# dhansmair/flamingo-mini

Hardware: AMD Instinct MI355X
Metric: images/sec (fwd+bwd) flamingo-mini bs=32 (higher is better)
Workload: dtype bf16

## Files before the change

### flamingo-mini_amd/csrc/ff_rowwise.hip

```cpp
#include "ff_common.h"
#include "ff_internal.h"

namespace ff {

#ifdef FF_XA_TIMELINE
__device__ unsigned long long g_ln_timeline[4096 * 8];
#define FF_LTL(i) do { if (threadIdx.x == 0 && blockIdx.x < 4096) g_ln_timeline[blockIdx.x * 8 + (i)] = __builtin_amdgcn_s_memrealtime(); } while (0)
#else
#define FF_LTL(i) do { } while (0)
#endif

template <typename T, int VEC> FF_DEV void ld(const T* p, float (&o)[VEC]) {
    if constexpr (VEC == 1) o[0] = to_f32(p[0]);
    else Vec<T>::load(p, o);
}
template <typename T, int VEC> FF_DEV void st(T* p, const float (&o)[VEC]) {
    if constexpr (VEC == 1) p[0] = from_f32<T>(o[0]);
    else Vec<T>::store(p, o);
}

template <typename T, int VEC>
__global__ __launch_bounds__(256) void ln_fwd_kernel(const LnArgs a_in, const T* __restrict__ x, const T* __restrict__ add,
                                                     const T* __restrict__ gamma, const T* __restrict__ beta, T* __restrict__ y,
                                                     float* __restrict__ mean, float* __restrict__ rstd) {
    const LnArgs a = fetch_args(a_in);
    pin_args(x, add, gamma, beta, y, mean, rstd);
    const int lane = threadIdx.x & 63;
    const int row = blockIdx.x * 4 + (threadIdx.x >> 6);
    if (row >= a.rows) return;
    const T* xr = x + a.x_map.off(row);
    const T* ar = nullptr;
    if (add) ar = add + (long long)((row % a.add_rows_per_seg) / a.add_div) * a.cols;
    const int nchunk = a.cols / VEC;
    float mu, rs;
    if (nchunk <= 4 * 64 && VEC > 1) {
        float v[4][VEC];
#pragma unroll
        for (int u = 0; u < 4; u++) {
            const int c = lane + 64 * u;
            if (c < nchunk) {
                ld<T, VEC>(xr + c * VEC, v[u]);
                if (ar) {
                    float t[VEC];
                    ld<T, VEC>(ar + c * VEC, t);
#pragma unroll
                    for (int i = 0; i < VEC; i++) v[u][i] += t[i];
                }
            }
        }
        if (a.stats_given) {
            mu = mean[row];
            rs = rstd[row];
        } else {
            float s = 0.f;
#pragma unroll
            for (int u = 0; u < 4; u++)
                if (lane + 64 * u < nchunk)
#pragma unroll
                    for (int i = 0; i < VEC; i++) s += v[u][i];
            mu = wave_sum(s) / (float)a.cols;
            float q = 0.f;
#pragma unroll
            for (int u = 0; u < 4; u++)
                if (lane + 64 * u < nchunk)
#pragma unroll
                    for (int i = 0; i < VEC; i++) q += (v[u][i] - mu) * (v[u][i] - mu);
            rs = rsqrtf(wave_sum(q) / (float)a.cols + a.eps);
            if (lane == 0 && mean) {
                mean[row] = mu;
                rstd[row] = rs;
            }
        }
        if (!y) return;
        T* yr = y + a.y_map.off(row);
#pragma unroll
        for (int u = 0; u < 4; u++) {
            const int c = lane + 64 * u;
            if (c < nchunk) {
                float g[VEC], b[VEC], o[VEC];
                ld<T, VEC>(gamma + c * VEC, g);
                ld<T, VEC>(beta + c * VEC, b);
#pragma unroll
                for (int i = 0; i < VEC; i++) o[i] = (v[u][i] - mu) * rs * g[i] + b[i];
                st<T, VEC>(yr + c * VEC, o);
            }
        }
        return;
    }
    if (a.stats_given) {
        mu = mean[row];
        rs = rstd[row];
    } else {
        float s = 0.f;
        for (int c = lane; c < nchunk; c += 64) {
            float v[VEC];
            ld<T, VEC>(xr + c * VEC, v);
            if (ar) {
                float t[VEC];
                ld<T, VEC>(ar + c * VEC, t);
#pragma unroll
                for (int i = 0; i < VEC; i++) v[i] += t[i];
            }
#pragma unroll
            for (int i = 0; i < VEC; i++) s += v[i];
        }
        mu = wave_sum(s) / (float)a.cols;
        float q = 0.f;
        for (int c = lane; c < nchunk; c += 64) {
            float v[VEC];
            ld<T, VEC>(xr + c * VEC, v);
            if (ar) {
                float t[VEC];
                ld<T, VEC>(ar + c * VEC, t);
#pragma unroll
                for (int i = 0; i < VEC; i++) v[i] += t[i];
            }
#pragma unroll
            for (int i = 0; i < VEC; i++) q += (v[i] - mu) * (v[i] - mu);
        }
        rs = rsqrtf(wave_sum(q) / (float)a.cols + a.eps);
        if (lane == 0 && mean) {
            mean[row] = mu;
            rstd[row] = rs;
        }
    }
    if (!y) return;
    T* yr = y + a.y_map.off(row);
    for (int c = lane; c < nchunk; c += 64) {
        float v[VEC], g[VEC], b[VEC];
        ld<T, VEC>(xr + c * VEC, v);
        if (ar) {
            float t[VEC];
            ld<T, VEC>(ar + c * VEC, t);
#pragma unroll
            for (int i = 0; i < VEC; i++) v[i] += t[i];
        }
        ld<T, VEC>(gamma + c * VEC, g);
        ld<T, VEC>(beta + c * VEC, b);
#pragma unroll
        for (int i = 0; i < VEC; i++) v[i] = (v[i] - mu) * rs * g[i] + b[i];
        st<T, VEC>(yr + c * VEC, v);
    }
}

template <typename T, int VEC>
__global__ __launch_bounds__(256) void ln_bwd_dx_kernel(const LnArgs a_in, const T* __restrict__ dy, const T* __restrict__ x,
                                                        const T* __restrict__ add, const T* __restrict__ gamma,
                                                        const float* __restrict__ mean, const float* __restrict__ rstd, T* dx,
                                                        const T* dx_res) {
    const LnArgs a = fetch_args(a_in);
    pin_args(dy, x, add, gamma, mean, rstd, dx, dx_res);
    const int lane = threadIdx.x & 63;
    const int row = blockIdx.x * 4 + (threadIdx.x >> 6);
    if (row >= a.rows) return;
    const T* xr = x + a.x_map.off(row);
    const T* dyr = dy + a.y_map.off(row);
    const T* ar = nullptr;
    if (add) ar = add + (long long)((row % a.add_rows_per_seg) / a.add_div) * a.cols;
    const float mu = mean[row], rs = rstd[row];
    const int nchunk = a.cols / VEC;
    float s1 = 0.f, s2 = 0.f;
    for (int c = lane; c < nchunk; c += 64) {
        float v[VEC], d[VEC], g[VEC];
        ld<T, VEC>(xr + c * VEC, v);
        if (ar) {
            float t[VEC];
            ld<T, VEC>(ar + c * VEC, t);
#pragma unroll
            for (int i = 0; i < VEC; i++) v[i] += t[i];
        }
        ld<T, VEC>(dyr + c * VEC, d);
        ld<T, VEC>(gamma + c * VEC, g);
#pragma unroll
        for (int i = 0; i < VEC; i++) {
            const float dyh = d[i] * g[i];
            s1 += dyh;
            s2 += dyh * (v[i] - mu) * rs;
        }
    }
    const float m1 = wave_sum(s1) / (float)a.cols, m2 = wave_sum(s2) / (float)a.cols;
    const long long doff = a.dx_map.off(row);
    for (int c = lane; c < nchunk; c += 64) {
        float v[VEC], d[VEC], g[VEC], o[VEC];
        ld<T, VEC>(xr + c * VEC, v);
        if (ar) {
            float t[VEC];
            ld<T, VEC>(ar + c * VEC, t);
#pragma unroll
            for (int i = 0; i < VEC; i++) v[i] += t[i];
        }
        ld<T, VEC>(dyr + c * VEC, d);
        ld<T, VEC>(gamma + c * VEC, g);
#pragma unroll
        for (int i = 0; i < VEC; i++) o[i] = rs * (d[i] * g[i] - m1 - (v[i] - mu) * rs * m2);
        if (dx_res) {
            float q[VEC];
            ld<T, VEC>(dx_res + doff + c * VEC, q);
#pragma unroll
            for (int i = 0; i < VEC; i++) o[i] += q[i];
        }
        st<T, VEC>(dx + doff + c * VEC, o);
    }
}


template <typename T, int VEC, int NCH>
__global__ __launch_bounds__(256) void ln_bwd_fused_kernel(const LnArgs a_in, const T* __restrict__ dy, const T* __restrict__ x,
                                                           const T* __restrict__ add, const T* __restrict__ gamma,
                                                           const float* __restrict__ mean, const float* __restrict__ rstd, T* dx,
                                                           const T* dx_res, const T* __restrict__ dot_a, const T* __restrict__ dot_b,
                                                           float* __restrict__ partial, int rows_per_block) {
    FF_LTL(0);
    const LnArgs a = fetch_args(a_in);
    pin_args(dy, x, add, gamma, mean, rstd, dx, dx_res, dot_a, dot_b, partial, rows_per_block);
    extern __shared__ __attribute__((aligned(16))) float sacc[];
    FF_LTL(1);
    __shared__ float red[4];
    const int lane = threadIdx.x & 63, w = threadIdx.x >> 6;
    const int nchunk = a.cols / VEC;
    float accg[NCH][VEC], accb[NCH][VEC];
#pragma unroll
    for (int i = 0; i < NCH; i++)
#pragma unroll
        for (int e = 0; e < VEC; e++) accg[i][e] = accb[i][e] = 0.f;
    float da = 0.f, db = 0.f;
    const int row_end = min(a.rows, (int)(blockIdx.x + 1) * rows_per_block);
    auto load_dy = [&](int row, const T* dyr, int c, float (&d)[VEC]) {
        if (a.dy_splits > 0) {
            const float* pp = (const float*)dy + (long long)row * a.cols + c * VEC;
#pragma unroll
            for (int e = 0; e < VEC; e++) d[e] = 0.f;
            for (int sp = 0; sp < a.dy_splits; sp++) {
#pragma unroll
                for (int e = 0; e < VEC; e += 4) {
                    const f32x4 q = *(const f32x4*)(pp + (long long)sp * a.dy_slab + e);
                    d[e] += q[0]; d[e + 1] += q[1]; d[e + 2] += q[2]; d[e + 3] += q[3];
                }
            }
        } else ld<T, VEC>(dyr + c * VEC, d);
    };
    for (int row = blockIdx.x * rows_per_block + w; row < row_end; row += 4) {
        const T* xr = x + a.x_map.off(row);
        const T* dyr = a.dy_splits > 0 ? dy : dy + a.y_map.off(row);
        const T* ar = add ? add + (long long)((row % a.add_rows_per_seg) / a.add_div) * a.cols : nullptr;
        const float mu = mean[row], rs = rstd[row];
        float s1 = 0.f, s2 = 0.f;
        constexpr bool KEEP = NCH <= 4;
        constexpr bool HOIST = KEEP && VEC > 1;
        float xk[KEEP ? NCH : 1][VEC], dk[KEEP ? NCH : 1][VEC];
        uint4 rq[HOIST ? NCH : 1], ra[HOIST ? NCH : 1], rb[HOIST ? NCH : 1];
        const long long doff = a.dx_map.off(row);
#pragma unroll
        for (int i = 0; i < NCH; i++) {
            const int c = lane + 64 * i;
            if (c < nchunk) {
                float v[VEC], d[VEC], g[VEC];
                ld<T, VEC>(xr + c * VEC, v);
                if (ar) {
                    float t[VEC];
                    ld<T, VEC>(ar + c * VEC, t);
#pragma unroll
                    for (int e = 0; e < VEC; e++) v[e] += t[e];
                }
                load_dy(row, dyr, c, d);
                ld<T, VEC>(gamma + c * VEC, g);
                if constexpr (HOIST) {
                    if (dx_res) rq[i] = *(const uint4*)(dx_res + doff + c * VEC);
                    if (dot_a) ra[i] = *(const uint4*)(dot_a + doff + c * VEC);
                    if (dot_b) rb[i] = *(const uint4*)(dot_b + doff + c * VEC);
                }
#pragma unroll
                for (int e = 0; e < VEC; e++) {
                    const float dyh = d[e] * g[e], xh = (v[e] - mu) * rs;
                    s1 += dyh;
                    s2 += dyh * xh;
                    if (KEEP) { xk[i][e] = xh; dk[i][e] = d[e]; }
                }
            }
        }
        const float m1 = wave_sum(s1) / (float)a.cols, m2 = wave_sum(s2) / (float)a.cols;
        auto unpack = [](const uint4& r, float (&o)[VEC]) {
            if constexpr (VEC > 1) {
                typedef typename Vec<T>::raw raw_t;
                const raw_t x = __builtin_bit_cast(raw_t, r);
#pragma unroll
                for (int e = 0; e < VEC; e++) o[e] = to_f32(x[e]);
            }
        };
#pragma unroll
        for (int i = 0; i < NCH; i++) {
            const int c = lane + 64 * i;
            if (c < nchunk) {
                float xh[VEC], d[VEC], g[VEC], o[VEC];
                if (KEEP) {
#pragma unroll
                    for (int e = 0; e < VEC; e++) { xh[e] = xk[i][e]; d[e] = dk[i][e]; }
                } else {
                    float v[VEC];
                    ld<T, VEC>(xr + c * VEC, v);
                    if (ar) {
                        float t[VEC];
                        ld<T, VEC>(ar + c * VEC, t);
#pragma unroll
                        for (int e = 0; e < VEC; e++) v[e] += t[e];
                    }
                    load_dy(row, dyr, c, d);
#pragma unroll
                    for (int e = 0; e < VEC; e++) xh[e] = (v[e] - mu) * rs;
                }
                ld<T, VEC>(gamma + c * VEC, g);
#pragma unroll
                for (int e = 0; e < VEC; e++) {
                    o[e] = rs * (d[e] * g[e] - m1 - xh[e] * m2);
                    accg[i][e] += d[e] * xh[e];
                    accb[i][e] += d[e];
                }
                if (dx_res) {
                    float q[VEC];
                    if constexpr (HOIST) unpack(rq[i], q);
                    else ld<T, VEC>(dx_res + doff + c * VEC, q);
                    if (dot_a) {
                        float u[VEC];
                        if constexpr (HOIST) unpack(ra[i], u);
                        else ld<T, VEC>(dot_a + doff + c * VEC, u);
#pragma unroll
                        for (int e = 0; e < VEC; e++) da += q[e] * u[e];
                    }
#pragma unroll
                    for (int e = 0; e < VEC; e++) o[e] += q[e];
                }
                if (dx) {
                    float r[VEC];
#pragma unroll
                    for (int e = 0; e < VEC; e++) r[e] = to_f32(from_f32<T>(o[e]));
                    if (dot_b) {
                        float u[VEC];
                        if constexpr (HOIST) unpack(rb[i], u);
                        else ld<T, VEC>(dot_b + doff + c * VEC, u);
#pragma unroll
                        for (int e = 0; e < VEC; e++) db += r[e] * u[e];
                    }
                    st<T, VEC>(dx + doff + c * VEC, o);
                }
            }
        }
    }
    FF_LTL(2);
    {
        float* mine = sacc + (size_t)w * 2 * a.cols;
#pragma unroll
        for (int i = 0; i < NCH; i++) {
            const int c = lane + 64 * i;
            if (c < nchunk) {
#pragma unroll
                for (int e = 0; e < VEC; e += 4) {
                    *(f32x4*)(mine + c * VEC + e) = f32x4{accg[i][e], accg[i][e + 1], accg[i][e + 2], accg[i][e + 3]};
                    *(f32x4*)(mine + a.cols + c * VEC + e) = f32x4{accb[i][e], accb[i][e + 1], accb[i][e + 2], accb[i][e + 3]};
                }
            }
        }
    }
    __syncthreads();
    FF_LTL(3);
    const long long P = 2LL * a.cols + 2;
    float* out = partial + (long long)blockIdx.x * P;
    for (int i = threadIdx.x * 4; i < 2 * a.cols; i += 256 * 4) {
        const f32x4 s0 = *(const f32x4*)(sacc + i), s1 = *(const f32x4*)(sacc + 2 * a.cols + i);
        const f32x4 s2 = *(const f32x4*)(sacc + 4 * a.cols + i), s3 = *(const f32x4*)(sacc + 6 * a.cols + i);
        float* o = out + i;
        o[0] = (s0[0] + s1[0]) + (s2[0] + s3[0]); o[1] = (s0[1] + s1[1]) + (s2[1] + s3[1]);
        o[2] = (s0[2] + s1[2]) + (s2[2] + s3[2]); o[3] = (s0[3] + s1[3]) + (s2[3] + s3[3]);
    }
    da = block_sum<4>(da, red);
    db = block_sum<4>(db, red);
    if (threadIdx.x == 0) { out[2 * a.cols] = da; out[2 * a.cols + 1] = db; }
    FF_LTL(4);
}

template <typename T>
FF_DEV void ln_final_body(int nblk, int cols, const float* __restrict__ partial, T* dgamma, T* dbeta, const T* alpha_a, T* out_a, const T* alpha_b,
                          T* out_b) {
    __shared__ float red[16][17];
    const int P = 2 * cols + 2;
    const int tx = threadIdx.x & 15, ty = threadIdx.x >> 4;
    const int idx = blockIdx.x * 16 + tx;
    float v[8] = {0.f, 0.f, 0.f, 0.f, 0.f, 0.f, 0.f, 0.f};
    if (idx < P) {
        int b = ty;
        for (; b + 7 * 16 < nblk; b += 8 * 16) {
#pragma unroll
            for (int u = 0; u < 8; u++) v[u] += partial[(long long)(b + 16 * u) * P + idx];
        }
        for (; b < nblk; b += 16) v[0] += partial[(long long)b * P + idx];
    }
    red[ty][tx] = ((v[0] + v[1]) + (v[2] + v[3])) + ((v[4] + v[5]) + (v[6] + v[7]));
    __syncthreads();
    if (ty == 0 && idx < P) {
        float s = 0.f;
#pragma unroll
        for (int u = 0; u < 16; u++) s += red[u][tx];
        const float v = s;
        if (idx < cols) { if (dgamma) dgamma[idx] = from_f32<T>(v); }
        else if (idx < 2 * cols) { if (dbeta) dbeta[idx - cols] = from_f32<T>(v); }
        else if (idx == 2 * cols) {
            if (out_a) { const float t = tanhf(to_f32(alpha_a[0])); out_a[0] = from_f32<T>(v * (1.f - t * t)); }
        } else if (out_b) { const float t = tanhf(to_f32(alpha_b[0])); out_b[0] = from_f32<T>(v * (1.f - t * t)); }
    }
}
template <typename T>
__global__ __launch_bounds__(256) void ln_bwd_final_kernel(int nblk, int cols, const float* __restrict__ partial, T* dgamma, T* dbeta,
                                                           const T* alpha_a, T* out_a, const T* alpha_b, T* out_b) {
    pin_args(nblk, cols, partial, dgamma, dbeta, alpha_a, out_a, alpha_b, out_b);
    ln_final_body<T>(nblk, cols, partial, dgamma, dbeta, alpha_a, out_a, alpha_b, out_b);
}
struct LnFinishTable {
    LnPending s[kLnFinishMax];
};
template <typename T>
__global__ __launch_bounds__(256) void ln_bwd_final_multi_kernel(const LnFinishTable t) {
    const LnPending& e = t.s[blockIdx.y];
    if ((int)blockIdx.x * 16 >= 2 * e.cols + 2) return;
    ln_final_body<T>(e.nblk, e.cols, e.partial, (T*)e.dgamma, (T*)e.dbeta, (const T*)e.alpha_a, (T*)e.out_a, (const T*)e.alpha_b, (T*)e.out_b);
}

struct ColReduceArgs {
    int rows, cols;
// ... 131 lines not shown

int gate_grad(int dtype, int rows, int cols, const void* a, const void* b, const void* alpha, void* dalpha, void* ws,
              size_t ws_bytes, hipStream_t st_);

static bool vec_ok(int dtype, int cols, std::initializer_list<RowMap> maps, std::initializer_list<const void*> ptrs) {
    const int n = dtype == FF_DTYPE_BF16 ? 8 : 4;
    if (cols % n) return false;
    for (const RowMap& m : maps)
        if (m.ld % n || (m.rows_per_seg > 0 && m.seg_stride % n)) return false;
    for (const void* p : ptrs)
        if (p && (uintptr_t)p % 16) return false;
    return true;
}

#define FF_DISPATCH_T_VEC(dtype, vec, ...)                 \
    do {                                                    \
        if ((dtype) == FF_DTYPE_BF16) {                     \
            typedef bf16 T;                                 \
            if (vec) { constexpr int VEC = 8; __VA_ARGS__; }       \
            else { constexpr int VEC = 1; __VA_ARGS__; }           \
        } else {                                            \
            typedef float T;                                \
            if (vec) { constexpr int VEC = 4; __VA_ARGS__; }       \
            else { constexpr int VEC = 1; __VA_ARGS__; }           \
        }                                                   \
    } while (0)

int layernorm_fwd(const LnArgs& a, const void* x, const void* add, const void* gamma, const void* beta, void* y, float* mean,
                  float* rstd, hipStream_t st_) {
    FF_CHECK(a.rows > 0 && a.cols > 0 && x, FF_ERR_SHAPE, "layernorm_fwd: bad shape rows=%d cols=%d", a.rows, a.cols);
    FF_CHECK(!a.stats_given || (mean && rstd), FF_ERR_SHAPE, "layernorm_fwd: stats_given without statistics");
    FF_CHECK(!y || (gamma && beta), FF_ERR_SHAPE, "layernorm_fwd: gamma/beta missing");
    FF_CHECK(!add || (a.add_rows_per_seg > 0 && a.add_div > 0), FF_ERR_SHAPE, "layernorm_fwd: addend needs add_rows_per_seg/add_div");
    const bool v = vec_ok(a.dtype, a.cols, {a.x_map, a.y_map}, {x, add, gamma, beta, y});
    const int grid = cdiv(a.rows, 4);
    FF_DISPATCH_T_VEC(a.dtype, v, ln_fwd_kernel<T, VEC><<<dim3(grid), dim3(256), 0, st_>>>(a, (const T*)x, (const T*)add, (const T*)gamma, (const T*)beta, (T*)y, mean, rstd));
    return check_launch("ln_fwd");
}

static void split_plan(int n_rows_in_group, int col_blocks, int ngroups, int& rows_per_split, int& nsplit) {
    int target = std::max(1, 512 / std::max(1, col_blocks * ngroups));
    nsplit = std::max(1, std::min(std::min(target, 32), cdiv(n_rows_in_group, 32)));
    rows_per_split = cdiv(n_rows_in_group, nsplit);
    nsplit = cdiv(n_rows_in_group, rows_per_split);
}

static size_t col_reduce_ws(int n_rows_in_group, int cols, int ngroups, int nslots) {
    int rps, ns;
    split_plan(n_rows_in_group, 1, ngroups, rps, ns);
    return (size_t)ns * ngroups * nslots * cols * sizeof(float);
}


static int ln_fused_blocks(int rows, int& rows_per_block) {
    rows_per_block = std::max(4, (cdiv(rows, 256) + 3) / 4 * 4);
    return cdiv(rows, rows_per_block);
}
static bool ln_fused_ok(int dtype, int cols, bool vec) {
    if (!vec) return false;
    const int n = dtype == FF_DTYPE_BF16 ? 8 : 4;
    return cdiv(cols / n, 64) <= 8 && (size_t)8 * cols * sizeof(float) <= 150 * 1024;
}
size_t layernorm_bwd_workspace(int rows, int cols) {
    int rpb;
    const size_t fused = (size_t)ln_fused_blocks(rows, rpb) * (2 * (size_t)cols + 2) * sizeof(float);
    return std::max(fused, col_reduce_ws(rows, cols, 1, 2));
}

bool layernorm_bwd_deferrable(int dtype, int cols) { return cols % (dtype == FF_DTYPE_BF16 ? 8 : 4) == 0 && ln_fused_ok(dtype, cols, true); }
int layernorm_bwd_partial_blocks(int rows) {
    int rpb;
    return ln_fused_blocks(rows, rpb);
}
size_t layernorm_bwd_partial_bytes(int rows, int cols) { return (size_t)layernorm_bwd_partial_blocks(rows) * (2 * (size_t)cols + 2) * sizeof(float); }

template <typename T, int VEC>
static int launch_ln_fused(const LnArgs& a, const void* dy, const void* x, const void* add, const void* gamma, const float* mean,
                           const float* rstd, void* dx, const void* dx_res, const LnDots& dots, void* dgamma, void* dbeta, float* partial,
                           hipStream_t st_, LnPending* pending) {
    int rpb;
    const int nblk = ln_fused_blocks(a.rows, rpb);
    const int nch = cdiv(a.cols / VEC, 64);
    const size_t lds = (size_t)8 * a.cols * sizeof(float);
#define FF_LN_LAUNCH(NCH)                                                                                                                 \
    do {                                                                                                                                  \
        if (lds > 48 * 1024) {                                                                                                            \
            static bool attr[64] = {};                                                                                                    \
            int dev = 0;                                                                                                                  \
            (void)hipGetDevice(&dev);                                                                                                     \
            if (dev < 0 || dev >= 64 || !attr[dev]) {                                                                                     \
                hipFuncSetAttribute((const void*)ln_bwd_fused_kernel<T, VEC, NCH>, hipFuncAttributeMaxDynamicSharedMemorySize, 150 * 1024); \
                if (dev >= 0 && dev < 64) attr[dev] = true;                                                                               \
            }                                                                                                                             \
        }                                                                                                                                 \
        ln_bwd_fused_kernel<T, VEC, NCH><<<dim3(nblk), dim3(256), lds, st_>>>(a, (const T*)dy, (const T*)x, (const T*)add, (const T*)gamma, \
                                                                              mean, rstd, (T*)dx, (const T*)dx_res, (const T*)dots.a,     \
                                                                              (const T*)dots.b, partial, rpb);                            \
    } while (0)
    if (nch <= 2) FF_LN_LAUNCH(2);
    else if (nch <= 4) FF_LN_LAUNCH(4);
    else FF_LN_LAUNCH(8);
#undef FF_LN_LAUNCH
    FF_TRY(check_launch("ln_bwd_fused"));
    if (pending) {
        pending->partial = partial; pending->nblk = nblk; pending->cols = a.cols; pending->dgamma = dgamma; pending->dbeta = dbeta;
        pending->alpha_a = dots.alpha_a; pending->out_a = dots.out_a; pending->alpha_b = dots.alpha_b; pending->out_b = dots.out_b;
        return FF_OK;
    }
    const int P = 2 * a.cols + 2;
    ln_bwd_final_kernel<T><<<dim3(cdiv(P, 16)), dim3(256), 0, st_>>>(nblk, a.cols, partial, (T*)dgamma, (T*)dbeta, (const T*)dots.alpha_a,
                                                                     (T*)dots.out_a, (const T*)dots.alpha_b, (T*)dots.out_b);
    return check_launch("ln_bwd_final");
}

int layernorm_bwd(const LnArgs& a, const void* dy, const void* x, const void* add, const void* gamma, const float* mean,
                  const float* rstd, void* dx, const void* dx_residual, void* dgamma, void* dbeta, void* ws, size_t ws_bytes,
                  hipStream_t st_, const LnDots* dots_in, LnPending* pending) {
    FF_CHECK(a.rows > 0 && a.cols > 0 && dy && x && gamma && mean && rstd, FF_ERR_SHAPE, "layernorm_bwd: null/shape");
    if (pending) *pending = LnPending{};
    FF_CHECK(!add || (a.add_rows_per_seg > 0 && a.add_div > 0), FF_ERR_SHAPE, "layernorm_bwd: addend needs add_rows_per_seg/add_div");
    const LnDots dots = dots_in ? *dots_in : LnDots{};
    FF_CHECK(!dots.a || dx_residual, FF_ERR_SHAPE, "layernorm_bwd: dot_a is taken against dx_residual");
    FF_CHECK(!dots.b || dx, FF_ERR_SHAPE, "layernorm_bwd: dot_b is taken against dx");
    const bool v = vec_ok(a.dtype, a.cols, {a.x_map, a.y_map, a.dx_map}, {x, add, gamma, dy, dx, dx_residual, dots.a, dots.b});
    FF_CHECK(a.dy_splits == 0 || (ln_fused_ok(a.dtype, a.cols, v) && (dgamma || dots.a || dots.b) && a.cols % 4 == 0), FF_ERR_UNSUPPORTED,
             "layernorm_bwd: summing split-K slabs needs the one-pass kernel");
    if (ln_fused_ok(a.dtype, a.cols, v) && (dgamma || dots.a || dots.b)) {
        FF_CHECK(!dgamma == !dbeta, FF_ERR_SHAPE, "layernorm_bwd: dgamma and dbeta come together");
        int rpb;
        const size_t need = (size_t)ln_fused_blocks(a.rows, rpb) * (2 * (size_t)a.cols + 2) * sizeof(float);
        FF_CHECK(ws && ws_bytes >= need, FF_ERR_WORKSPACE, "layernorm_bwd workspace: need %zu have %zu", need, ws_bytes);
        if (a.dtype == FF_DTYPE_BF16) return launch_ln_fused<bf16, 8>(a, dy, x, add, gamma, mean, rstd, dx, dx_residual, dots, dgamma, dbeta, (float*)ws, st_, pending);
        return launch_ln_fused<float, 4>(a, dy, x, add, gamma, mean, rstd, dx, dx_residual, dots, dgamma, dbeta, (float*)ws, st_, pending);
    }
    if (dots.a) FF_TRY(gate_grad(a.dtype, a.rows, a.cols, dx_residual, dots.a, dots.alpha_a, dots.out_a, ws, ws_bytes, st_));
    if (dx) {
        const int grid = cdiv(a.rows, 4);
        FF_DISPATCH_T_VEC(a.dtype, v, ln_bwd_dx_kernel<T, VEC><<<dim3(grid), dim3(256), 0, st_>>>(a, (const T*)dy, (const T*)x, (const T*)add, (const T*)gamma, mean, rstd, (T*)dx, (const T*)dx_residual));
        FF_TRY(check_launch("ln_bwd_dx"));
    }
    if (dgamma || dbeta) {
        FF_CHECK(dgamma && dbeta, FF_ERR_SHAPE, "layernorm_bwd: dgamma and dbeta come together");
        const int vecn = v ? (a.dtype == FF_DTYPE_BF16 ? 8 : 4) : 1;
        ColReduceArgs c = {};
        c.rows = a.rows; c.cols = a.cols; c.x_map = a.x_map; c.y_map = a.y_map;
        c.rows_per_batch = a.rows; c.rows_per_group = a.rows; c.n_batch = 1; c.ngroups = 1;
        c.add_rows_per_seg = a.add_rows_per_seg; c.add_div = a.add_div;
        const int col_blocks = cdiv(a.cols, 64 * vecn);
        split_plan(a.rows, col_blocks, 1, c.rows_per_split, c.nsplit);
        const size_t need = (size_t)c.nsplit * 2 * a.cols * sizeof(float);
        FF_CHECK(ws && ws_bytes >= need, FF_ERR_WORKSPACE, "layernorm_bwd workspace: need %zu have %zu", need, ws_bytes);
        FF_DISPATCH_T_VEC(a.dtype, v, col_reduce_kernel<T, VEC, 1><<<dim3(col_blocks, 1, c.nsplit), dim3(256), 0, st_>>>(c, (const T*)x, (const T*)dy, (const T*)add, mean, rstd, (float*)ws));
        FF_TRY(check_launch("ln_bwd_param_partial"));
        const int grid = std::min(cdiv(2LL * a.cols, 256), 1024);
        if (a.dtype == FF_DTYPE_BF16)
            hipLaunchKernelGGL(col_reduce_final_kernel<bf16>, dim3(grid), dim3(256), 0, st_, c.nsplit, 1, 2, a.cols, (const float*)ws, (bf16*)dgamma, (bf16*)dbeta);
        else
            hipLaunchKernelGGL(col_reduce_final_kernel<float>, dim3(grid), dim3(256), 0, st_, c.nsplit, 1, 2, a.cols, (const float*)ws, (float*)dgamma, (float*)dbeta);
        FF_TRY(check_launch("ln_bwd_param_final"));
    }
    if (dots.b) FF_TRY(gate_grad(a.dtype, a.rows, a.cols, dx, dots.b, dots.alpha_b, dots.out_b, ws, ws_bytes, st_));
    return FF_OK;
}

int layernorm_bwd_finish(int dtype, const LnPending* sets, int n, hipStream_t st_) {
    for (int i0 = 0; i0 < n; i0 += kLnFinishMax) {
        LnFinishTable t = {};
        int cnt = 0, pmax = 0;
        for (int i = i0; i < n && i < i0 + kLnFinishMax; i++)
            if (sets[i].partial) {
                t.s[cnt++] = sets[i];
                pmax = std::max(pmax, 2 * sets[i].cols + 2);
            }
        if (!cnt) continue;
        const dim3 grid(cdiv(pmax, 16), cnt);
        if (dtype == FF_DTYPE_BF16) ln_bwd_final_multi_kernel<bf16><<<grid, dim3(256), 0, st_>>>(t);
        else ln_bwd_final_multi_kernel<float><<<grid, dim3(256), 0, st_>>>(t);
        FF_TRY(check_launch("ln_bwd_final_multi"));
    }
    return FF_OK;
}

size_t rows_reduce_workspace(int rows, int cols, int rows_per_batch, int rows_per_group) {
    if (rows_per_batch <= 0 || rows_per_group <= 0) return 0;
// ... 115 lines not shown
```

Measured before the change: 782.3.

## Use buffer loads with OOB masking and batched prefetch in layernorm kernels

```diff
diff --git a/flamingo-mini_amd/csrc/ff_rowwise.hip b/flamingo-mini_amd/csrc/ff_rowwise.hip
--- a/flamingo-mini_amd/csrc/ff_rowwise.hip
+++ b/flamingo-mini_amd/csrc/ff_rowwise.hip
@@ -19,12 +19,160 @@
     else Vec<T>::store(p, o);
 }
 
+typedef __attribute__((ext_vector_type(4))) unsigned u32x4;
+constexpr unsigned kRowOob = 0x80000000u;
+FF_DEV __amdgpu_buffer_rsrc_t row_rsrc(const void* p, bool there = true) { return __builtin_amdgcn_make_buffer_rsrc((void*)p, 0, there ? 0x7fffffff : 0, 0x00020000); }
+FF_DEV u32x4 row_ld(__amdgpu_buffer_rsrc_t r, unsigned byte_off) { return __builtin_amdgcn_raw_buffer_load_b128(r, byte_off, 0, 0); }
+FF_DEV float row_ld_f32(__amdgpu_buffer_rsrc_t r, unsigned byte_off) { return __builtin_bit_cast(float, __builtin_amdgcn_raw_buffer_load_b32(r, byte_off, 0, 0)); }
+FF_DEV int wave_id() { return __builtin_amdgcn_readfirstlane(threadIdx.x >> 6); }
+template <typename T, int VEC> FF_DEV void unpk(const u32x4& r, float (&o)[VEC]) {
+    typedef typename Vec<T>::raw raw_t;
+    const raw_t x = __builtin_bit_cast(raw_t, r);
+#pragma unroll
+    for (int e = 0; e < VEC; e++) o[e] = to_f32(x[e]);
+}
+template <typename T, int VEC> FF_DEV void row_st(__amdgpu_buffer_rsrc_t r, unsigned byte_off, const float (&o)[VEC]) {
+    typename Vec<T>::raw v;
+#pragma unroll
+    for (int e = 0; e < VEC; e++) v[e] = from_f32<T>(o[e]);
+    __builtin_amdgcn_raw_buffer_store_b128(__builtin_bit_cast(u32x4, v), r, byte_off, 0, 0);
+}
+template <typename T, int VEC> FF_DEV void ldb(__amdgpu_buffer_rsrc_t r, int c, float (&o)[VEC]) { unpk<T, VEC>(row_ld(r, (unsigned)c * 16u), o); }
+
+template <typename T, int VEC>
+FF_DEV void ln_fwd_vec(const LnArgs& a, const T* x, const T* add, const T* gamma, const T* beta, T* y, float* mean, float* rstd) {
+    const int lane = threadIdx.x & 63;
+    const int row = blockIdx.x * 4 + wave_id();
+    if (row >= a.rows) return;
+    const bool has_add = add != nullptr;
+    const __amdgpu_buffer_rsrc_t rx = row_rsrc(x + a.x_map.off(row));
+    const __amdgpu_buffer_rsrc_t ra = row_rsrc(add + (long long)((row % (has_add ? a.add_rows_per_seg : 1)) / (has_add ? a.add_div : 1)) * a.cols, has_add);
+    const __amdgpu_buffer_rsrc_t rg = row_rsrc(gamma, y != nullptr), rb = row_rsrc(beta, y != nullptr);
+    const int nchunk = a.cols / VEC;
+    float mu, rs;
+    if (nchunk <= 4 * 64) {
+        u32x4 px[4], pa[4], pg[4], pb[4];
+        bool in[4];
+        unsigned coff[4];
+#pragma unroll
+        for (int u = 0; u < 4; u++) {
+            in[u] = lane + 64 * u < nchunk;
+            coff[u] = in[u] ? (unsigned)(lane + 64 * u) * 16u : kRowOob;
+            px[u] = row_ld(rx, coff[u]);
+        }
+#pragma unroll
+        for (int u = 0; u < 4; u++) pa[u] = row_ld(ra, coff[u]);
+        const float mu_in = row_ld_f32(row_rsrc(mean, a.stats_given != 0), (unsigned)row * 4u);
+        const float rs_in = row_ld_f32(row_rsrc(rstd, a.stats_given != 0), (unsigned)row * 4u);
+#pragma unroll
+        for (int u = 0; u < 4; u++) {
+            pg[u] = row_ld(rg, coff[u]);
+            pb[u] = row_ld(rb, coff[u]);
+        }
+        __builtin_amdgcn_sched_barrier(0);
+        asm volatile("" ::"v"(mu_in), "v"(rs_in));
+        float v[4][VEC];
+#pragma unroll
+        for (int u = 0; u < 4; u++) {
+            float t[VEC];
+            unpk<T, VEC>(px[u], v[u]);
+            unpk<T, VEC>(pa[u], t);
+#pragma unroll
+            for (int i = 0; i < VEC; i++) v[u][i] = has_add ? v[u][i] + t[i] : v[u][i];
+        }
+        if (a.stats_given) {
+            mu = mu_in;
+            rs = rs_in;
+        } else {
+            float s = 0.f;
+#pragma unroll
+            for (int u = 0; u < 4; u++)
+#pragma unroll
+                for (int i = 0; i < VEC; i++) s += v[u][i];
+            mu = wave_sum(s) / (float)a.cols;
+            float q = 0.f;
+#pragma unroll
+            for (int u = 0; u < 4; u++) {
+                const float mu_u = in[u] ? mu : 0.f;
+#pragma unroll
+                for (int i = 0; i < VEC; i++) q += (v[u][i] - mu_u) * (v[u][i] - mu_u);
+            }
+            rs = rsqrtf(wave_sum(q) / (float)a.cols + a.eps);
+            if (lane == 0 && mean) {
+                mean[row] = mu;
+                rstd[row] = rs;
+            }
+        }
+        if (!y) return;
+        const __amdgpu_buffer_rsrc_t ry = row_rsrc(y + a.y_map.off(row));
+#pragma unroll
+        for (int u = 0; u < 4; u++) {
+            float g[VEC], b[VEC], o[VEC];
+            unpk<T, VEC>(pg[u], g);
+            unpk<T, VEC>(pb[u], b);
+#pragma unroll
+            for (int i = 0; i < VEC; i++) o[i] = (v[u][i] - mu) * rs * g[i] + b[i];
+            if (in[u]) row_st<T, VEC>(ry, coff[u], o);
+        }
+        return;
+    }
+    auto load_x = [&](int c, float (&v)[VEC]) {
+        ldb<T, VEC>(rx, c, v);
+        if (has_add) {
+            float t[VEC];
+            ldb<T, VEC>(ra, c, t);
+#pragma unroll
+            for (int i = 0; i < VEC; i++) v[i] += t[i];
+        }
+    };
+    if (a.stats_given) {
+        mu = row_ld_f32(row_rsrc(mean), (unsigned)row * 4u);
+        rs = row_ld_f32(row_rsrc(rstd), (unsigned)row * 4u);
+    } else {
+        float s = 0.f;
+        for (int c = lane; c < nchunk; c += 64) {
+            float v[VEC];
+            load_x(c, v);
+#pragma unroll
+            for (int i = 0; i < VEC; i++) s += v[i];
+        }
+        mu = wave_sum(s) / (float)a.cols;
+        float q = 0.f;
+        for (int c = lane; c < nchunk; c += 64) {
+            float v[VEC];
+            load_x(c, v);
+#pragma unroll
+            for (int i = 0; i < VEC; i++) q += (v[i] - mu) * (v[i] - mu);
+        }
+        rs = rsqrtf(wave_sum(q) / (float)a.cols + a.eps);
+        if (lane == 0 && mean) {
+            mean[row] = mu;
+            rstd[row] = rs;
+        }
+    }
+    if (!y) return;
+    const __amdgpu_buffer_rsrc_t ry = row_rsrc(y + a.y_map.off(row));
+    for (int c = lane; c < nchunk; c += 64) {
+        float v[VEC], g[VEC], b[VEC];
+        load_x(c, v);
+        ldb<T, VEC>(rg, c, g);
+        ldb<T, VEC>(rb, c, b);
+#pragma unroll
+        for (int i = 0; i < VEC; i++) v[i] = (v[i] - mu) * rs * g[i] + b[i];
+        row_st<T, VEC>(ry, (unsigned)c * 16u, v);
+    }
+}
+
 template <typename T, int VEC>
 __global__ __launch_bounds__(256) void ln_fwd_kernel(const LnArgs a_in, const T* __restrict__ x, const T* __restrict__ add,
                                                      const T* __restrict__ gamma, const T* __restrict__ beta, T* __restrict__ y,
                                                      float* __restrict__ mean, float* __restrict__ rstd) {
     const LnArgs a = fetch_args(a_in);
     pin_args(x, add, gamma, beta, y, mean, rstd);
+    if constexpr (VEC > 1) {
+        ln_fwd_vec<T, VEC>(a, x, add, gamma, beta, y, mean, rstd);
+        return;
+    }
     const int lane = threadIdx.x & 63;
     const int row = blockIdx.x * 4 + (threadIdx.x >> 6);
     if (row >= a.rows) return;
@@ -33,60 +181,6 @@
     if (add) ar = add + (long long)((row % a.add_rows_per_seg) / a.add_div) * a.cols;
     const int nchunk = a.cols / VEC;
     float mu, rs;
-    if (nchunk <= 4 * 64 && VEC > 1) {
-        float v[4][VEC];
-#pragma unroll
-        for (int u = 0; u < 4; u++) {
-            const int c = lane + 64 * u;
-            if (c < nchunk) {
-                ld<T, VEC>(xr + c * VEC, v[u]);
-                if (ar) {
-                    float t[VEC];
-                    ld<T, VEC>(ar + c * VEC, t);
-#pragma unroll
-                    for (int i = 0; i < VEC; i++) v[u][i] += t[i];
-                }
-            }
-        }
-        if (a.stats_given) {
-            mu = mean[row];
-            rs = rstd[row];
-        } else {
-            float s = 0.f;
-#pragma unroll
-            for (int u = 0; u < 4; u++)
-                if (lane + 64 * u < nchunk)
-#pragma unroll
-                    for (int i = 0; i < VEC; i++) s += v[u][i];
-            mu = wave_sum(s) / (float)a.cols;
-            float q = 0.f;
-#pragma unroll
-            for (int u = 0; u < 4; u++)
-                if (lane + 64 * u < nchunk)
-#pragma unroll
-                    for (int i = 0; i < VEC; i++) q += (v[u][i] - mu) * (v[u][i] - mu);
-            rs = rsqrtf(wave_sum(q) / (float)a.cols + a.eps);
-            if (lane == 0 && mean) {
-                mean[row] = mu;
-                rstd[row] = rs;
-            }
-        }
-        if (!y) return;
-        T* yr = y + a.y_map.off(row);
-#pragma unroll
-        for (int u = 0; u < 4; u++) {
-            const int c = lane + 64 * u;
-            if (c < nchunk) {
-                float g[VEC], b[VEC], o[VEC];
-                ld<T, VEC>(gamma + c * VEC, g);
-                ld<T, VEC>(beta + c * VEC, b);
-#pragma unroll
-                for (int i = 0; i < VEC; i++) o[i] = (v[u][i] - mu) * rs * g[i] + b[i];
-                st<T, VEC>(yr + c * VEC, o);
-            }
-        }
-        return;
-    }
     if (a.stats_given) {
         mu = mean[row];
         rs = rstd[row];
@@ -150,6 +244,50 @@
                                                         const T* dx_res) {
     const LnArgs a = fetch_args(a_in);
     pin_args(dy, x, add, gamma, mean, rstd, dx, dx_res);
+    if constexpr (VEC > 1) {
+        const int lane = threadIdx.x & 63;
+        const int row = blockIdx.x * 4 + wave_id();
+        if (row >= a.rows) return;
+        const bool has_add = add != nullptr, has_res = dx_res != nullptr;
+        const __amdgpu_buffer_rsrc_t rx = row_rsrc(x + a.x_map.off(row)), rdy = row_rsrc(dy + a.y_map.off(row)), rg = row_rsrc(gamma);
+        const __amdgpu_buffer_rsrc_t ra = row_rsrc(add + (long long)((row % (has_add ? a.add_rows_per_seg : 1)) / (has_add ? a.add_div : 1)) * a.cols, has_add);
+        const long long doff = a.dx_map.off(row);
+        const __amdgpu_buffer_rsrc_t rq = row_rsrc(dx_res + doff, has_res), ro = row_rsrc(dx + doff);
+        const float mu = row_ld_f32(row_rsrc(mean), (unsigned)row * 4u), rs = row_ld_f32(row_rsrc(rstd), (unsigned)row * 4u);
+        const int nchunk = a.cols / VEC;
+        float s1 = 0.f, s2 = 0.f;
+        for (int c = lane; c < nchunk; c += 64) {
+            float v[VEC], t[VEC], d[VEC], g[VEC];
+            ldb<T, VEC>(rx, c, v);
+            ldb<T, VEC>(ra, c, t);
+            ldb<T, VEC>(rdy, c, d);
+            ldb<T, VEC>(rg, c, g);
+#pragma unroll
+            for (int i = 0; i < VEC; i++) {
+                v[i] = has_add ? v[i] + t[i] : v[i];
+                const float dyh = d[i] * g[i];
+                s1 += dyh;
+                s2 += dyh * (v[i] - mu) * rs;
+            }
+        }
+        const float m1 = wave_sum(s1) / (float)a.cols, m2 = wave_sum(s2) / (float)a.cols;
+        for (int c = lane; c < nchunk; c += 64) {
+            float v[VEC], t[VEC], d[VEC], g[VEC], q[VEC], o[VEC];
+            ldb<T, VEC>(rx, c, v);
+            ldb<T, VEC>(ra, c, t);
+            ldb<T, VEC>(rdy, c, d);
+            ldb<T, VEC>(rg, c, g);
+            ldb<T, VEC>(rq, c, q);
+#pragma unroll
+            for (int i = 0; i < VEC; i++) {
+                v[i] = has_add ? v[i] + t[i] : v[i];
+                o[i] = rs * (d[i] * g[i] - m1 - (v[i] - mu) * rs * m2);
+                o[i] = has_res ? o[i] + q[i] : o[i];
+            }
+            row_st<T, VEC>(ro, (unsigned)c * 16u, o);
+        }
+        return;
+    }
     const int lane = threadIdx.x & 63;
     const int row = blockIdx.x * 4 + (threadIdx.x >> 6);
     if (row >= a.rows) return;
@@ -204,7 +342,14 @@
 }
 
 
-template <typename T, int VEC, int NCH>
+constexpr int kLnSlabMax = 8;
+template <int VEC, int G, int SL> struct LnRowRegs {
+    static constexpr int ND = SL > 0 ? G * SL * (VEC / 4) : G;
+    u32x4 x[G], ad[G], g[G], q[G], ua[G], ub[G];
+    u32x4 dy[ND];
+    float mu, rs;
+};
+template <typename T, int VEC, int NCH, int SL>
 __global__ __launch_bounds__(256) void ln_bwd_fused_kernel(const LnArgs a_in, const T* __restrict__ dy, const T* __restrict__ x,
                                                            const T* __restrict__ add, const T* __restrict__ gamma,
                                                            const float* __restrict__ mean, const float* __restrict__ rstd, T* dx,
@@ -216,7 +361,7 @@
     extern __shared__ __attribute__((aligned(16))) float sacc[];
     FF_LTL(1);
     __shared__ float red[4];
-    const int lane = threadIdx.x & 63, w = threadIdx.x >> 6;
+    const int lane = threadIdx.x & 63, w = wave_id();
     const int nchunk = a.cols / VEC;
     float accg[NCH][VEC], accb[NCH][VEC];
 #pragma unroll
@@ -225,123 +370,174 @@
         for (int e = 0; e < VEC; e++) accg[i][e] = accb[i][e] = 0.f;
     float da = 0.f, db = 0.f;
     const int row_end = min(a.rows, (int)(blockIdx.x + 1) * rows_per_block);
-    auto load_dy = [&](int row, const T* dyr, int c, float (&d)[VEC]) {
-        if (a.dy_splits > 0) {
-            const float* pp = (const float*)dy + (long long)row * a.cols + c * VEC;
+    const bool has_add = add != nullptr, has_res = dx_res != nullptr;
+    constexpr int G = NCH <= 4 ? NCH : SL > 0 ? 1 : 2;
+    constexpr bool KEEP = G == NCH;
+    constexpr bool DB = NCH == 2 && SL == 0;
+    typedef LnRowRegs<VEC, G, SL> Regs;
+    bool in[NCH];
+    unsigned coff[NCH], soff[NCH];
+#pragma unroll
+    for (int i = 0; i < NCH; i++) {
+        in[i] = lane + 64 * i < nchunk;
+        coff[i] = in[i] ? (unsigned)(lane + 64 * i) * 16u : kRowOob;
+        soff[i] = in[i] ? (unsigned)(lane + 64 * i) * (VEC * 4u) : kRowOob;
+    }
+    const __amdgpu_buffer_rsrc_t rmean = row_rsrc(mean), rrstd = row_rsrc(rstd), rgam = row_rsrc(gamma);
+    u32x4 pg[KEEP ? NCH : 1];
+    if constexpr (KEEP)
+#pragma unroll
+        for (int i = 0; i < NCH; i++) pg[i] = row_ld(rgam, coff[i]);
+    auto issue = [&](Regs& R, int row_in, bool ok, int i0, bool second) {
+        const int row = ok ? row_in : 0;
+        const long long doff = a.dx_map.off(row);
+        const __amdgpu_buffer_rsrc_t rx = row_rsrc(x + a.x_map.off(row), ok);
+        const __amdgpu_buffer_rsrc_t ra = row_rsrc(add + (long long)((row % (has_add ? a.add_rows_per_seg : 1)) / (has_add ? a.add_div : 1)) * a.cols, ok && has_add);
+#pragma unroll
+        for (int j = 0; j < G; j++) R.x[j] = row_ld(rx, coff[i0 + j]);
+#pragma unroll
+        for (int j = 0; j < G; j++) R.ad[j] = row_ld(ra, coff[i0 + j]);
+        if constexpr (SL > 0) {
+            const float* pp = (const float*)dy + (long long)row * a.cols;
+#pragma unroll
+            for (int sp = 0; sp < SL; sp++) {
+                const __amdgpu_buffer_rsrc_t rs_ = row_rsrc(pp + (long long)sp * a.dy_slab, ok && sp < a.dy_splits);
+#pragma unroll
+                for (int j = 0; j < G; j++)
+#pragma unroll
+                    for (int h = 0; h < VEC / 4; h++) R.dy[(j * SL + sp) * (VEC / 4) + h] = row_ld(rs_, soff[i0 + j] + 16u * h);
+            }
+        } else {
+            const __amdgpu_buffer_rsrc_t rdy = row_rsrc(dy + a.y_map.off(row), ok);
+#pragma unroll
+            for (int j = 0; j < G; j++) R.dy[j] = row_ld(rdy, coff[i0 + j]);
+        }
+        if constexpr (!KEEP)
+#pragma unroll
+            for (int j = 0; j < G; j++) R.g[j] = row_ld(rgam, coff[i0 + j]);
+        R.mu = row_ld_f32(rmean, (unsigned)row * 4u);
+        R.rs = row_ld_f32(rrstd, (unsigned)row * 4u);
+        if (second) {
+            const __amdgpu_buffer_rsrc_t rq = row_rsrc(dx_res + doff, ok && has_res);
+            const __amdgpu_buffer_rsrc_t rua = row_rsrc(dot_a + doff, ok && dot_a), rub = row_rsrc(dot_b + doff, ok && dot_b);
+#pragma unroll
+            for (int j = 0; j < G; j++) R.q[j] = row_ld(rq, coff[i0 + j]);
+#pragma unroll
+            for (int j = 0; j < G; j++) R.ua[j] = row_ld(rua, coff[i0 + j]);
+#pragma unroll
+            for (int j = 0; j < G; j++) R.ub[j] = row_ld(rub, coff[i0 + j]);
+        }
+    };
+    auto operands = [&](const Regs& R, int row, int j, int i, float (&xh)[VEC], float (&d)[VEC], float (&g)[VEC]) {
+        float v[VEC], t[VEC];
+        unpk<T, VEC>(R.x[j], v);
+        unpk<T, VEC>(R.ad[j], t);
+        if constexpr (SL > 0) {
 #pragma unroll
             for (int e = 0; e < VEC; e++) d[e] = 0.f;
-            for (int sp = 0; sp < a.dy_splits; sp++) {
+#pragma unroll
+            for (int sp = 0; sp < SL; sp++)
 #pragma unroll
                 for (int e = 0; e < VEC; e += 4) {
-                    const f32x4 q = *(const f32x4*)(pp + (long long)sp * a.dy_slab + e);
+                    const f32x4 q = __builtin_bit_cast(f32x4, R.dy[(j * SL + sp) * (VEC / 4) + e / 4]);
                     d[e] += q[0]; d[e + 1] += q[1]; d[e + 2] += q[2]; d[e + 3] += q[3];
                 }
-            }
-        } else ld<T, VEC>(dyr + c * VEC, d);
+            if ((SL == kLnSlabMax || NCH > 4) && a.dy_splits > SL && in[i]) {
+                const float* pp = (const float*)dy + (long long)row * a.cols + (lane + 64 * i) * VEC;
+                for (int sp = SL; sp < a.dy_splits; sp++)
+#pragma unroll
+                    for (int e = 0; e < VEC; e += 4) {
+                        const f32x4 q = *(const __attribute__((address_space(1))) f32x4*)(pp + (long long)sp * a.dy_slab + e);
+                        d[e] += q[0]; d[e + 1] += q[1]; d[e + 2] += q[2]; d[e + 3] += q[3];
+                    }
+            }
+        } else unpk<T, VEC>(R.dy[j], d);
+        unpk<T, VEC>(KEEP ? pg[KEEP ? i : 0] : R.g[j], g);
+        const float mu_i = in[i] ? R.mu : 0.f, rs_i = in[i] ? R.rs : 0.f;
+#pragma unroll
+        for (int e = 0; e < VEC; e++) {
+            v[e] = has_add ? v[e] + t[e] : v[e];
+            xh[e] = (v[e] - mu_i) * rs_i;
+        }
     };
-    for (int row = blockIdx.x * rows_per_block + w; row < row_end; row += 4) {
-        const T* xr = x + a.x_map.off(row);
-        const T* dyr = a.dy_splits > 0 ? dy : dy + a.y_map.off(row);
-        const T* ar = add ? add + (long long)((row % a.add_rows_per_seg) / a.add_div) * a.cols : nullptr;
-        const float mu = mean[row], rs = rstd[row];
+    auto finish = [&](const Regs& R, __amdgpu_buffer_rsrc_t ro, int j, int i, float rs, float m1, float m2, const float (&xh)[VEC],
+                      const float (&d)[VEC], const float (&g)[VEC]) {
+        float o[VEC], q[VEC], u[VEC], r[VEC];
+#pragma unroll
+        for (int e = 0; e < VEC; e++) {
+            o[e] = rs * (d[e] * g[e] - m1 - xh[e] * m2);
+            accg[i][e] += d[e] * xh[e];
+            accb[i][e] += d[e];
+        }
+        unpk<T, VEC>(R.q[j], q);
+        unpk<T, VEC>(R.ua[j], u);
+#pragma unroll
+        for (int e = 0; e < VEC; e++) da += q[e] * u[e];
+#pragma unroll
+        for (int e = 0; e < VEC; e++) o[e] = has_res ? o[e] + q[e] : o[e];
+#pragma unroll
+        for (int e = 0; e < VEC; e++) r[e] = to_f32(from_f32<T>(o[e]));
+        unpk<T, VEC>(R.ub[j], u);
+#pragma unroll
+        for (int e = 0; e < VEC; e++) db += r[e] * u[e];
+        if (in[i] && dx) row_st<T, VEC>(ro, coff[i], o);
+    };
+    const int row0 = blockIdx.x * rows_per_block + w;
+    Regs cur;
+    if constexpr (DB) issue(cur, row0, row0 < row_end, 0, true);
+    for (int row = row0; row < row_end; row += 4) {
         float s1 = 0.f, s2 = 0.f;
-        constexpr bool KEEP = NCH <= 4;
-        constexpr bool HOIST = KEEP && VEC > 1;
-        float xk[KEEP ? NCH : 1][VEC], dk[KEEP ? NCH : 1][VEC];
-        uint4 rq[HOIST ? NCH : 1], ra[HOIST ? NCH : 1], rb[HOIST ? NCH : 1];
-        const long long doff = a.dx_map.off(row);
-#pragma unroll
-        for (int i = 0; i < NCH; i++) {
-            const int c = lane + 64 * i;
-            if (c < nchunk) {
-                float v[VEC], d[VEC], g[VEC];
-                ld<T, VEC>(xr + c * VEC, v);
-                if (ar) {
-                    float t[VEC];
-                    ld<T, VEC>(ar + c * VEC, t);
-#pragma unroll
-                    for (int e = 0; e < VEC; e++) v[e] += t[e];
+        const __amdgpu_buffer_rsrc_t ro = row_rsrc(dx + a.dx_map.off(row), dx != nullptr);
+        if constexpr (KEEP) {
+            Regs nxt;
+            if constexpr (DB) issue(nxt, row + 4, row + 4 < row_end, 0, true);
+            else issue(cur, row, true, 0, true);
+            __builtin_amdgcn_sched_barrier(0);
+            float xk[NCH][VEC], dk[NCH][VEC], g[NCH][VEC];
+#pragma unroll
+            for (int i = 0; i < NCH; i++) {
+                operands(cur, row, i, i, xk[i], dk[i], g[i]);
+#pragma unroll
+                for (int e = 0; e < VEC; e++) {
+                    const float dyh = dk[i][e] * g[i][e];
+                    s1 += dyh;
+                    s2 += dyh * xk[i][e];
                 }
-                load_dy(row, dyr, c, d);
-                ld<T, VEC>(gamma + c * VEC, g);
-                if constexpr (HOIST) {
-                    if (dx_res) rq[i] = *(const uint4*)(dx_res + doff + c * VEC);
-                    if (dot_a) ra[i] = *(const uint4*)(dot_a + doff + c * VEC);
-                    if (dot_b) rb[i] = *(const uint4*)(dot_b + doff + c * VEC);
+            }
+            const float m1 = wave_sum(s1) / (float)a.cols, m2 = wave_sum(s2) / (float)a.cols;
+#pragma unroll
+            for (int i = 0; i < NCH; i++) finish(cur, ro, i, i, cur.rs, m1, m2, xk[i], dk[i], g[i]);
+            if constexpr (DB) cur = nxt;
+        } else {
+            float rs = 0.f;
+#pragma unroll
+            for (int i0 = 0; i0 < NCH; i0 += G) {
+                issue(cur, row, true, i0, false);
+#pragma unroll
+                for (int j = 0; j < G; j++) {
+                    float xh[VEC], d[VEC], g[VEC];
+                    operands(cur, row, j, i0 + j, xh, d, g);
+#pragma unroll
+                    for (int e = 0; e < VEC; e++) {
+                        const float dyh = d[e] * g[e];
+                        s1 += dyh;
+                        s2 += dyh * xh[e];
+                    }
                 }
-#pragma unroll
-                for (int e = 0; e < VEC; e++) {
-                    const float dyh = d[e] * g[e], xh = (v[e] - mu) * rs;
-                    s1 += dyh;
-                    s2 += dyh * xh;
-                    if (KEEP) { xk[i][e] = xh; dk[i][e] = d[e]; }
+                rs = cur.rs;
+                if constexpr (SL > 0) __builtin_amdgcn_sched_barrier(0);
+            }
+            const float m1 = wave_sum(s1) / (float)a.cols, m2 = wave_sum(s2) / (float)a.cols;
+#pragma unroll
+            for (int i0 = 0; i0 < NCH; i0 += G) {
+                issue(cur, row, true, i0, true);
+#pragma unroll
+                for (int j = 0; j < G; j++) {
+                    float xh[VEC], d[VEC], g[VEC];
+                    operands(cur, row, j, i0 + j, xh, d, g);
+                    finish(cur, ro, j, i0 + j, rs, m1, m2, xh, d, g);
                 }
-            }
-        }
-        const float m1 = wave_sum(s1) / (float)a.cols, m2 = wave_sum(s2) / (float)a.cols;
-        auto unpack = [](const uint4& r, float (&o)[VEC]) {
-            if constexpr (VEC > 1) {
-                typedef typename Vec<T>::raw raw_t;
-                const raw_t x = __builtin_bit_cast(raw_t, r);
-#pragma unroll
-                for (int e = 0; e < VEC; e++) o[e] = to_f32(x[e]);
-            }
-        };
-#pragma unroll
-        for (int i = 0; i < NCH; i++) {
-            const int c = lane + 64 * i;
-            if (c < nchunk) {
-                float xh[VEC], d[VEC], g[VEC], o[VEC];
-                if (KEEP) {
-#pragma unroll
-                    for (int e = 0; e < VEC; e++) { xh[e] = xk[i][e]; d[e] = dk[i][e]; }
-                } else {
-                    float v[VEC];
-                    ld<T, VEC>(xr + c * VEC, v);
-                    if (ar) {
-                        float t[VEC];
-                        ld<T, VEC>(ar + c * VEC, t);
-#pragma unroll
-                        for (int e = 0; e < VEC; e++) v[e] += t[e];
-                    }
-                    load_dy(row, dyr, c, d);
-#pragma unroll
-                    for (int e = 0; e < VEC; e++) xh[e] = (v[e] - mu) * rs;
-                }
-                ld<T, VEC>(gamma + c * VEC, g);
-#pragma unroll
-                for (int e = 0; e < VEC; e++) {
-                    o[e] = rs * (d[e] * g[e] - m1 - xh[e] * m2);
-                    accg[i][e] += d[e] * xh[e];
-                    accb[i][e] += d[e];
-                }
-                if (dx_res) {
-                    float q[VEC];
-                    if constexpr (HOIST) unpack(rq[i], q);
-                    else ld<T, VEC>(dx_res + doff + c * VEC, q);
-                    if (dot_a) {
-                        float u[VEC];
-                        if constexpr (HOIST) unpack(ra[i], u);
-                        else ld<T, VEC>(dot_a + doff + c * VEC, u);
-#pragma unroll
-                        for (int e = 0; e < VEC; e++) da += q[e] * u[e];
-                    }
-#pragma unroll
-                    for (int e = 0; e < VEC; e++) o[e] += q[e];
-                }
-                if (dx) {
-                    float r[VEC];
-#pragma unroll
-                    for (int e = 0; e < VEC; e++) r[e] = to_f32(from_f32<T>(o[e]));
-                    if (dot_b) {
-                        float u[VEC];
-                        if constexpr (HOIST) unpack(rb[i], u);
-                        else ld<T, VEC>(dot_b + doff + c * VEC, u);
-#pragma unroll
-                        for (int e = 0; e < VEC; e++) db += r[e] * u[e];
-                    }
-                    st<T, VEC>(dx + doff + c * VEC, o);
-                }
+                if constexpr (SL > 0) __builtin_amdgcn_sched_barrier(0);
             }
         }
     }
@@ -639,24 +835,32 @@
     const int nblk = ln_fused_blocks(a.rows, rpb);
     const int nch = cdiv(a.cols / VEC, 64);
     const size_t lds = (size_t)8 * a.cols * sizeof(float);
-#define FF_LN_LAUNCH(NCH)                                                                                                                 \
+#define FF_LN_LAUNCH(NCH, SL)                                                                                                                \
     do {                                                                                                                                  \
         if (lds > 48 * 1024) {                                                                                                            \
             static bool attr[64] = {};                                                                                                    \
             int dev = 0;                                                                                                                  \
             (void)hipGetDevice(&dev);                                                                                                     \
             if (dev < 0 || dev >= 64 || !attr[dev]) {                                                                                     \
-                hipFuncSetAttribute((const void*)ln_bwd_fused_kernel<T, VEC, NCH>, hipFuncAttributeMaxDynamicSharedMemorySize, 150 * 1024); \
+                hipFuncSetAttribute((const void*)ln_bwd_fused_kernel<T, VEC, NCH, SL>, hipFuncAttributeMaxDynamicSharedMemorySize, 150 * 1024); \
                 if (dev >= 0 && dev < 64) attr[dev] = true;                                                                               \
             }                                                                                                                             \
         }                                                                                                                                 \
-        ln_bwd_fused_kernel<T, VEC, NCH><<<dim3(nblk), dim3(256), lds, st_>>>(a, (const T*)dy, (const T*)x, (const T*)add, (const T*)gamma, \
+        ln_bwd_fused_kernel<T, VEC, NCH, SL><<<dim3(nblk), dim3(256), lds, st_>>>(a, (const T*)dy, (const T*)x, (const T*)add, (const T*)gamma, \
                                                                               mean, rstd, (T*)dx, (const T*)dx_res, (const T*)dots.a,     \
                                                                               (const T*)dots.b, partial, rpb);                            \
     } while (0)
-    if (nch <= 2) FF_LN_LAUNCH(2);
-    else if (nch <= 4) FF_LN_LAUNCH(4);
-    else FF_LN_LAUNCH(8);
+#define FF_LN_LAUNCH_NCH(SL)            \
+    do {                                \
+        if (nch <= 2) FF_LN_LAUNCH(2, SL);      \
+        else if (nch == 3) FF_LN_LAUNCH(3, SL); \
+        else if (nch == 4) FF_LN_LAUNCH(4, SL); \
+        else FF_LN_LAUNCH(8, (SL > 4 ? 4 : SL)); \
+    } while (0)
+    if (a.dy_splits <= 0) FF_LN_LAUNCH_NCH(0);
+    else if (a.dy_splits <= 4) FF_LN_LAUNCH_NCH(4);
+    else FF_LN_LAUNCH_NCH(kLnSlabMax);
+#undef FF_LN_LAUNCH_NCH
 #undef FF_LN_LAUNCH
     FF_TRY(check_launch("ln_bwd_fused"));
     if (pending) {
```

After: 789.0, median of 6. No clear change (+0.9%).
